# hpcaitech/Open-Sora

Measured on NVIDIA H100. Metric: denoise-steps/sec STDiT3-XL/2 64x32x32 bf16, higher is better.
Workload: dtype bf16

## Files before the change

open-sora_b200/csrc/common.cuh:

```cuda
#pragma once

#include <cuda.h>
#include <cuda_bf16.h>
#include <cuda_runtime.h>
#include <stdint.h>
#include <stdio.h>

#include "../../include/osb200.h"

namespace osb {

void set_error(const char* fmt, ...);
void count_launch(int n = 1);
bool initialised();
int sm_count();

#define OSB_CHECK_CUDA(expr)                                                            \
  do {                                                                                  \
    cudaError_t _e = (expr);                                                            \
    if (_e != cudaSuccess) {                                                            \
      osb::set_error("%s failed: %s (%s:%d)", #expr, cudaGetErrorString(_e), __FILE__,  \
                     __LINE__);                                                         \
      return OSB_ERR_CUDA;                                                              \
    }                                                                                   \
// ... 192 lines not shown
                   reinterpret_cast<uint64_t>(m)),
               "r"(src), "r"(c0), "r"(c1)
               : "memory");
}
__device__ __forceinline__ void tma_store_5d(const CUtensorMap* m, uint32_t src, int32_t c0, int32_t c1, int32_t c2,
                                             int32_t c3, int32_t c4) {
  asm volatile("cp.async.bulk.tensor.5d.global.shared::cta.bulk_group [%0, {%2, %3, %4, %5, %6}], [%1];" ::"l"(
                   reinterpret_cast<uint64_t>(m)),
               "r"(src), "r"(c0), "r"(c1), "r"(c2), "r"(c3), "r"(c4)
               : "memory");
}
__device__ __forceinline__ void bulk_commit_group() { asm volatile("cp.async.bulk.commit_group;" ::: "memory"); }
__device__ __forceinline__ void bulk_wait_group_read_all() { asm volatile("cp.async.bulk.wait_group.read 0;" ::: "memory"); }
__device__ __forceinline__ void named_barrier_sync(uint32_t id, uint32_t count) {
  asm volatile("bar.sync %0, %1;" ::"r"(id), "r"(count) : "memory");
}
__device__ __forceinline__ void wgmma_fence() { asm volatile("wgmma.fence.sync.aligned;" ::: "memory"); }
__device__ __forceinline__ void wgmma_commit() { asm volatile("wgmma.commit_group.sync.aligned;" ::: "memory"); }
template <int N>
__device__ __forceinline__ void wgmma_wait() { asm volatile("wgmma.wait_group.sync.aligned %0;" ::"n"(N) : "memory"); }
template <int R>
__device__ __forceinline__ void wgmma_fence_regs(float (&d)[R]) {
#pragma unroll
  for (int i = 0; i < R; ++i) asm volatile("" : "+f"(d[i])::"memory");
}

__device__ __forceinline__ uint64_t make_sw128_kmajor_desc(uint32_t smem_addr) {
  uint64_t d = 0;
  d |= static_cast<uint64_t>((smem_addr & 0x3FFFF) >> 4);
  d |= static_cast<uint64_t>(1) << 16;
// ... 90 lines not shown
```

open-sora_b200/csrc/gemm_sm90.cu:

```cuda
#include <stdlib.h>

#include <type_traits>

#include "common.cuh"
#include "tiles.cuh"
#include "wgmma.cuh"

namespace osb {

constexpr int kBlockM = 128;
constexpr int kBlockK = 64;
constexpr int kNumThreads = 384;
constexpr int kStageBudget = 200 * 1024;
constexpr int kSmemLimit = 227 * 1024;

enum { kPlain = 0, kConv = 1, kHeadTiles = 2, kLora = 3, kText = 4, kFp8 = 5, kFp8Blk = 6 };

struct Fp8BlockParams {
  int64_t a_ld, a_kstride;
  uint8_t* d8;
  float* d_scale;
  int64_t ldd8, ld_dscale;
};

// ... 40 lines not shown
  static constexpr int B_BYTES = BLOCK_N * kBlockK * 2;
  static constexpr int STAGE_BYTES = A_BYTES + B_BYTES;
  static constexpr int EPI_BYTES = kStaged ? kBlockM * BLOCK_N * 2 : 0;
  static constexpr int RING_BUDGET = kStaged ? kSmemLimit - 1024 - 256 - EPI_BYTES : kStageBudget;
  static constexpr int STAGES_RAW = RING_BUDGET / STAGE_BYTES;
  static constexpr int STAGES = STAGES_RAW > 6 ? 6 : STAGES_RAW;
  static constexpr int NUM_BARS = 2 * STAGES + (kStaged ? 2 : 0);
  static constexpr int SMEM_BYTES = STAGES * STAGE_BYTES + EPI_BYTES + 1024 + 8 * NUM_BARS;
  static_assert(STAGES >= 2, "pipeline needs at least two stages");
  static_assert(SMEM_BYTES <= kSmemLimit, "shared memory");
  static_assert(B_BYTES % 1024 == 0, "W tile must keep 1024-byte swizzle-atom alignment");
  static_assert(BLOCK_N % 16 == 0 && BLOCK_N <= 256, "wgmma N");
  static_assert(!kStaged || BLOCK_N % 64 == 0, "the staged epilogue moves 64-column boxes");
};

template <int BLOCK_N, int kMode>
__global__ void __launch_bounds__(kNumThreads, 1)
gemm_bf16_kernel(const __grid_constant__ CUtensorMap tmap_a, const __grid_constant__ CUtensorMap tmap_w,
                 const GemmEpilogueParams p, const ConvGeom cg, const HeadTileParams ht,
                 const __grid_constant__ CUtensorMap tmap_u, const __grid_constant__ CUtensorMap tmap_lb,
                 const int32_t lora_k_blocks,
                 const float* a_scale, const float* w_scale,
                 const Fp8BlockParams fb,
                 const __grid_constant__ CUtensorMap tmap_r,
                 const __grid_constant__ CUtensorMap tmap_d) {
  constexpr bool kStaged = staged_epilogue(kMode);
  using Cfg = GemmCfg<BLOCK_N, kStaged>;
  constexpr int kStages = Cfg::STAGES;
  constexpr int kBK = (kMode == kFp8 || kMode == kFp8Blk) ? 2 * kBlockK : kBlockK;
  constexpr uint32_t kEpiBoxBytes = kBlockM * 128;

// ... 37 lines not shown
  if (threadIdx.x == 0) {
    tma_prefetch_desc(&tmap_a);
    tma_prefetch_desc(&tmap_w);
    if constexpr (kMode == kLora) {
      tma_prefetch_desc(&tmap_u);
      tma_prefetch_desc(&tmap_lb);
    }
    if constexpr (kStaged) {
      if (p.R != nullptr) tma_prefetch_desc(&tmap_r);
      tma_prefetch_desc(&tmap_d);
      mbar_init(res_bar, 1);
      mbar_init(epi_free, 1);
    }
    for (int s = 0; s < kStages; ++s) {
      mbar_init(full_bar(s), 1);
      mbar_init(empty_bar(s), 2);
    }
    fence_barrier_init();
  }
  __syncthreads();
  pdl_wait();

  if (wg == 0) {
    asm volatile("setmaxnreg.dec.sync.aligned.u32 40;\n" ::: "memory");
    if (tid_wg == 0) {
      int stage = 0;
      uint32_t phase = 0;
      uint32_t it = 0;
      for (int64_t t = blockIdx.x; t < num_tiles; t += gridDim.x, ++it) {
        const Tile tl = tile_at(t);
        const int32_t a_row = (int32_t)(tl.m_blk * kBlockM);
        const int32_t w_row = (int32_t)(tl.n_blk * BLOCK_N);
        auto load_k_block = [&](int64_t kb) {
          mbar_wait_notrace(empty_bar(stage), phase ^ 1);
          mbar_expect_tx(full_bar(stage), Cfg::STAGE_BYTES);
          if (kMode == kLora && kb >= num_k_blocks) {
            const int32_t lk0 = (int32_t)(kb - num_k_blocks) * kBlockK;
            tma_load_2d(&tmap_u, full_bar(stage), smem_a(stage), lk0, a_row);
            tma_load_2d(&tmap_lb, full_bar(stage), smem_b(stage), lk0, w_row);
// ... 2 lines not shown
            if constexpr (kMode == kConv) {
              const int tap = (int)(kb / cg.cin_chunks);
              const int32_t ac = (int32_t)(kb - (int64_t)tap * cg.cin_chunks) * kBlockK;
              const int32_t aw = tl.w0 * cg.sw + tap % cg.kw_n;
              const int32_t ah = tl.h0 * cg.sh + (tap / cg.kw_n) % cg.kh_n;
              const int32_t at = tl.t0 * cg.st + tap / (cg.kw_n * cg.kh_n);
              tma_load_5d(&tmap_a, full_bar(stage), smem_a(stage), ac, aw, ah, at, tl.n_i);
            } else {
              tma_load_2d(&tmap_a, full_bar(stage), smem_a(stage), k0, a_row);
            }
            tma_load_2d(&tmap_w, full_bar(stage), smem_b(stage), k0, w_row);
          }
          if (++stage == kStages) { stage = 0; phase ^= 1; }
        };
        int64_t kb = 0;
        if constexpr (kStaged) {
          if (p.R != nullptr) {
            for (; kb < min((int64_t)kStages, total_k_blocks); ++kb) load_k_block(kb);
            if (it > 0) mbar_wait_notrace(epi_free, (it - 1) & 1u);
            const int live = (int)min((int64_t)(BLOCK_N / 64), (p.N - w_row + 63) / 64);
            mbar_expect_tx(res_bar, (uint32_t)live * kEpiBoxBytes);
            for (int c = 0; c < live; ++c) {
              if constexpr (kMode == kConv)
                tma_load_5d(&tmap_r, res_bar, epi_base + c * kEpiBoxBytes, w_row + 64 * c, tl.w0, tl.h0, tl.t0, tl.n_i);
              else
                tma_load_2d(&tmap_r, res_bar, epi_base + c * kEpiBoxBytes, w_row + 64 * c, a_row);
            }
          }
        }
        for (; kb < total_k_blocks; ++kb) load_k_block(kb);
      }
      pdl_launch_dependents();
    }
    return;
  }

  asm volatile("setmaxnreg.inc.sync.aligned.u32 232;\n" ::: "memory");
  const int cw = wg - 1;
  int stage = 0;
  uint32_t phase = 0;
  uint32_t it = 0;
  auto release_epi_buffer = [&](int64_t kb) {
    if constexpr (kStaged) {
      if (kb == 0 && it > 0 && threadIdx.x == 128) {
        bulk_wait_group_read_all();
        mbar_arrive(epi_free);
      }
    }
  };
  for (int64_t t = blockIdx.x; t < num_tiles; t += gridDim.x, ++it) {
    const Tile tl = tile_at(t);
    const int64_t m_blk = tl.m_blk, n_blk = tl.n_blk;
    const int warp_in = tid_wg >> 5, lane = tid_wg & 31;
    const int r_frag = cw * 64 + warp_in * 16 + (lane >> 2);
    const int c_frag = 2 * (lane & 3);
    const float* gate_row[2] = {nullptr, nullptr};
    float sa[2] = {0.f, 0.f};
    if constexpr (kStaged && kMode != kConv) {
      const uint32_t group_rows32 = (uint32_t)(p.group_rows > 0xffffffffll ? 0xffffffffu : p.group_rows);
#pragma unroll
      for (int h = 0; h < 2; ++h) {
        const int64_t row = min(m_blk * kBlockM + r_frag + 8 * h, p.M - 1);
        if (p.epilogue == OSB_EPI_BIAS_GATE_RES && p.gate != nullptr) {
          int64_t gi = (uint32_t)row / group_rows32;
          if (p.mod_index) gi = p.mod_index[gi];
          gate_row[h] = p.gate + gi * p.gate_stride;
        }
        if constexpr (kMode == kFp8) sa[h] = __ldg(a_scale + row);
      }
    }
    float acc[BLOCK_N / 2];
#pragma unroll
    for (int i = 0; i < BLOCK_N / 2; ++i) acc[i] = 0.f;
    if constexpr (kMode == kFp8 || kMode == kFp8Blk) {
      float part[BLOCK_N / 2];
#pragma unroll
      for (int i = 0; i < BLOCK_N / 2; ++i) part[i] = 0.f;
      const float* sa_row0 = a_scale;
      const float* sa_row1 = a_scale;
      if constexpr (kMode == kFp8Blk) {
        const int64_t r0 = m_blk * kBlockM + cw * 64 + (tid_wg >> 5) * 16 + ((tid_wg & 31) >> 2);
        sa_row0 = a_scale + min(r0, p.M - 1) * fb.a_ld;
        sa_row1 = a_scale + min(r0 + 8, p.M - 1) * fb.a_ld;
      }
      for (int64_t kb = 0; kb < total_k_blocks; ++kb) {
        float s0 = 1.f, s1 = 1.f;
        if constexpr (kMode == kFp8Blk) {
          s0 = __ldg(sa_row0 + kb * fb.a_kstride);
          s1 = __ldg(sa_row1 + kb * fb.a_kstride);
// ... 2 lines not shown
        const uint64_t da = make_sw128_kmajor_desc(smem_a(stage) + (uint32_t)(cw * 64 * 128));
        const uint64_t db = make_sw128_kmajor_desc(smem_b(stage));
        wgmma_fence_regs(part);
        wgmma_fence();
#pragma unroll
        for (int k = 0; k < 4; ++k)
          WgmmaFp8<BLOCK_N>::mma(part, da + (uint64_t)(2 * k), db + (uint64_t)(2 * k), k > 0 ? 1u : 0u);
        wgmma_commit();
        release_epi_buffer(kb);
        wgmma_wait<0>();
        wgmma_fence_regs(part);
        if (tid_wg == 0) mbar_arrive(empty_bar(stage));
        if constexpr (kMode == kFp8Blk) {
#pragma unroll
          for (int j = 0; j < BLOCK_N / 8; ++j) {
            acc[4 * j] = fmaf(part[4 * j], s0, acc[4 * j]);
            acc[4 * j + 1] = fmaf(part[4 * j + 1], s0, acc[4 * j + 1]);
            acc[4 * j + 2] = fmaf(part[4 * j + 2], s1, acc[4 * j + 2]);
            acc[4 * j + 3] = fmaf(part[4 * j + 3], s1, acc[4 * j + 3]);
          }
        } else {
#pragma unroll
          for (int i = 0; i < BLOCK_N / 2; ++i) acc[i] += part[i];
        }
        if (++stage == kStages) { stage = 0; phase ^= 1; }
      }
    } else {
      int prev = 0;
      for (int64_t kb = 0; kb < total_k_blocks; ++kb) {
        mbar_wait_notrace(full_bar(stage), phase);
        const uint64_t da = make_sw128_kmajor_desc(smem_a(stage) + (uint32_t)(cw * 64 * 128));
        const uint64_t db = make_sw128_kmajor_desc(smem_b(stage));
        wgmma_fence_regs(acc);
        wgmma_fence();
#pragma unroll
        for (int k = 0; k < kBlockK / 16; ++k)
          Wgmma<BLOCK_N>::mma(acc, da + (uint64_t)(2 * k), db + (uint64_t)(2 * k), (kb > 0 || k > 0) ? 1u : 0u);
        wgmma_commit();
        release_epi_buffer(kb);
        wgmma_wait<1>();
        wgmma_fence_regs(acc);
        if (kb > 0 && tid_wg == 0) mbar_arrive(empty_bar(prev));
        prev = stage;
        if (++stage == kStages) { stage = 0; phase ^= 1; }
      }
      wgmma_wait<0>();
      wgmma_fence_regs(acc);
      if (tid_wg == 0) mbar_arrive(empty_bar(prev));
    }

    if constexpr (kMode == kLora) {
      if (w_scale != nullptr) {
#pragma unroll
        for (int j = 0; j < BLOCK_N / 8; ++j) {
          const int64_t n = min(n_blk * BLOCK_N + 8 * j + c_frag, p.N - 2);
          const float2 cs = __ldg(reinterpret_cast<const float2*>(w_scale + n));
          acc[4 * j] *= cs.x;
          acc[4 * j + 1] *= cs.y;
          acc[4 * j + 2] *= cs.x;
          acc[4 * j + 3] *= cs.y;
        }
      }
    }

    if constexpr (kMode == kFp8Blk && BLOCK_N == 128) {
      if (p.epilogue == OSB_EPI_BIAS_GELU_TANH_FP8) {
        const int64_t n0 = n_blk * BLOCK_N + c_frag;
#pragma unroll
        for (int h = 0; h < 2; ++h) {
          const int64_t row = m_blk * kBlockM + r_frag + 8 * h;
          float amax = 0.f;
#pragma unroll
          for (int j = 0; j < BLOCK_N / 8; ++j) {
            const int64_t n = n0 + 8 * j;
            const float2 sw = __ldg(reinterpret_cast<const float2*>(w_scale + n));
            float v0 = acc[4 * j + 2 * h] * sw.x, v1 = acc[4 * j + 2 * h + 1] * sw.y;
            if (p.bias) {
              const float2 b = unpack_bf16x2(__ldg(reinterpret_cast<const uint32_t*>(p.bias + n)));
              v0 += b.x;
              v1 += b.y;
            }
            v0 = gelu_tanh(v0);
            v1 = gelu_tanh(v1);
            acc[4 * j + 2 * h] = v0;
            acc[4 * j + 2 * h + 1] = v1;
            amax = fmaxf(amax, fmaxf(fabsf(v0), fabsf(v1)));
          }
          amax = fmaxf(amax, __shfl_xor_sync(0xffffffffu, amax, 1));
          amax = fmaxf(amax, __shfl_xor_sync(0xffffffffu, amax, 2));
          const float s = amax > 0.f ? amax / 448.0f : 1.0f;
          if (row < p.M) {
            uint8_t* drow = fb.d8 + row * fb.ldd8;
#pragma unroll
            for (int j = 0; j < BLOCK_N / 8; ++j)
              *reinterpret_cast<uint16_t*>(drow + n0 + 8 * j) =
                  (uint16_t)e4m3x2(acc[4 * j + 2 * h] / s, acc[4 * j + 2 * h + 1] / s);
            if (c_frag == 0) fb.d_scale[row * fb.ld_dscale + n_blk] = s;
          }
        }
        continue;
      }
    }

    if constexpr (kMode == kHeadTiles) {
      constexpr int D = BLOCK_N / 2;
      using HT = HeadTileCfg<D>;
      constexpr int JH = D / 8;
      const int C = ht.heads * D;
      const uint32_t chunk_bytes = (uint32_t)ht.map.TR * 128u;
#pragma unroll
      for (int h = 0; h < 2; ++h) {
        const int64_t row = m_blk * kBlockM + r_frag + 8 * h;
        const bool row_ok = row < p.M;
        uint32_t pos = 0, tile_i = 0;
        int r = 0;
        if (row_ok) tile_of_row(ht.map, (uint32_t)row, tile_i, pos, r);
#pragma unroll
        for (int hh = 0; hh < 2; ++hh) {
          const int64_t col0 = n_blk * BLOCK_N + hh * D;
          if (col0 >= p.N) continue;
          const int kidx = (int)((uint32_t)col0 / (uint32_t)C);
          const int head = (int)((uint32_t)col0 - (uint32_t)kidx * (uint32_t)C) / D;
          const int kind = kidx % ht.nkinds;
          float x[JH][2];
#pragma unroll
          for (int j = 0; j < JH; ++j) {
            x[j][0] = acc[4 * (hh * JH + j) + 2 * h];
            x[j][1] = acc[4 * (hh * JH + j) + 2 * h + 1];
            if (p.bias) {
              const float2 b = unpack_bf16x2(__ldg(reinterpret_cast<const uint32_t*>(p.bias + col0 + 8 * j + c_frag)));
              x[j][0] += b.x;
              x[j][1] += b.y;
            }
          }
          if ((ht.norm_mask >> kind) & 1u) {
            float ss = 0.f;
#pragma unroll
            for (int j = 0; j < JH; ++j) ss += x[j][0] * x[j][0] + x[j][1] * x[j][1];
            ss += __shfl_xor_sync(0xffffffffu, ss, 1);
            ss += __shfl_xor_sync(0xffffffffu, ss, 2);
            const float rs = rsqrtf(ss * (1.0f / D) + ht.eps);
            const __nv_bfloat16* w = kind == 0 ? ht.norm_w[0] : (kind == 1 ? ht.norm_w[1] : (kind == 2 ? ht.norm_w[2] : ht.norm_w[3]));
#pragma unroll
            for (int j = 0; j < JH; ++j) {
              const float2 f = unpack_bf16x2(__ldg(reinterpret_cast<const uint32_t*>(w + 8 * j + c_frag)));
              x[j][0] *= rs * f.x;
              x[j][1] *= rs * f.y;
            }
          }
          if ((ht.rope_mask >> kind) & 1u) {
#pragma unroll
            for (int j = 0; j < JH; ++j) {
              const int64_t i = (int64_t)pos * (D / 2) + (8 * j + c_frag) / 2;
              const float cc = __ldg(ht.cos + i), sn = __ldg(ht.sin + i);
              const float a = x[j][0], b = x[j][1];
              x[j][0] = a * cc - b * sn;
              x[j][1] = b * cc + a * sn;
            }
          }
          uint8_t* dst = ht.base + (int64_t)kidx * ht.kind_stride + (int64_t)head * ht.head_stride + (int64_t)tile_i * ht.tile_bytes;
          const bool odd = (lane & 1) != 0, high = (lane & 2) != 0;
#pragma unroll
          for (int j0 = 0; j0 < HT::MAIN * 8; j0 += 4) {
            uint32_t u0 = pack_bf16x2(x[j0][0], x[j0][1]), u1 = pack_bf16x2(x[j0 + 1][0], x[j0 + 1][1]);
            uint32_t u2 = pack_bf16x2(x[j0 + 2][0], x[j0 + 2][1]), u3 = pack_bf16x2(x[j0 + 3][0], x[j0 + 3][1]);
            uint32_t s0 = __shfl_xor_sync(0xffffffffu, odd ? u0 : u1, 1);
            uint32_t s1 = __shfl_xor_sync(0xffffffffu, odd ? u2 : u3, 1);
            if (odd) { u0 = s0; u2 = s1; } else { u1 = s0; u3 = s1; }
            s0 = __shfl_xor_sync(0xffffffffu, high ? u0 : u2, 2);
            s1 = __shfl_xor_sync(0xffffffffu, high ? u1 : u3, 2);
            if (high) { u0 = s0; u1 = s1; } else { u2 = s0; u3 = s1; }
            if (row_ok)
              *reinterpret_cast<uint4*>(dst + tile_unit_off<HT::MAIN>(r, j0 + (lane & 3), chunk_bytes)) = make_uint4(u0, u1, u2, u3);
          }
          if (!row_ok) continue;
#pragma unroll
          for (int j = HT::MAIN * 8; j < JH; ++j)
            *reinterpret_cast<uint32_t*>(dst + tile_unit_off<HT::MAIN>(r, j, chunk_bytes) + c_frag * 2) = pack_bf16x2(x[j][0], x[j][1]);
          if constexpr (HT::UP > HT::U)
            *reinterpret_cast<uint32_t*>(dst + tile_unit_off<HT::MAIN>(r, HT::U, chunk_bytes) + c_frag * 2) = 0u;
        }
      }
    } else if constexpr (kMode == kText) {
#pragma unroll
      for (int h = 0; h < 2; ++h) {
        const int64_t row = m_blk * kBlockM + r_frag + 8 * h;
        if (row >= p.M) continue;
        __nv_bfloat16* drow = p.D + row * p.ldd;
#pragma unroll
        for (int j = 0; j < BLOCK_N / 8; ++j) {
          const int64_t n = n_blk * BLOCK_N + 8 * j + c_frag;
          if (n >= p.N) continue;
          float v0 = acc[4 * j + 2 * h], v1 = acc[4 * j + 2 * h + 1];
          if (p.bias) {
            const float2 b = unpack_bf16x2(__ldg(reinterpret_cast<const uint32_t*>(p.bias + n)));
            v0 += b.x;
            v1 += b.y;
          }
          if (p.epilogue == OSB_EPI_GATED_GELU) {
            drow[n >> 1] = __float2bfloat16_rn(gelu_tanh(v0) * v1);
          } else {
            v0 = v0 / (1.0f + __expf(-1.702f * v0));
            v1 = v1 / (1.0f + __expf(-1.702f * v1));
            *reinterpret_cast<uint32_t*>(drow + n) = pack_bf16x2(v0, v1);
          }
        }
      }
    } else {
      static_assert(kStaged, "every other mode has its own epilogue");
      uint8_t* const epi = smem_raw + (epi_base - smem_u32(smem_raw));
      const bool gate_res = p.epilogue == OSB_EPI_BIAS_GATE_RES;
      if (!gate_res) gate_row[0] = gate_row[1] = nullptr;
      const bool has_res = gate_res && p.R != nullptr;
      if (p.R != nullptr)
        mbar_wait_notrace(res_bar, it & 1u);
      else if (it > 0)
        mbar_wait_notrace(epi_free, (it - 1) & 1u);
      auto body = [&](auto gelu) {
#pragma unroll
        for (int j = 0; j < BLOCK_N / 8; ++j) {
          const int64_t n = min(n_blk * BLOCK_N + 8 * j + c_frag, p.N - 2);
          float2 sw = make_float2(1.f, 1.f), b = make_float2(-0.f, -0.f);
          if constexpr (kMode == kFp8 || kMode == kFp8Blk) sw = __ldg(reinterpret_cast<const float2*>(w_scale + n));
          if (p.bias) b = unpack_bf16x2(__ldg(reinterpret_cast<const uint32_t*>(p.bias + n)));
#pragma unroll
          for (int h = 0; h < 2; ++h) {
            const int li = r_frag + 8 * h;
            uint32_t* const cell = reinterpret_cast<uint32_t*>(epi + (j >> 3) * kEpiBoxBytes + li * 128 +
                                                               (((j & 7) ^ (li & 7)) << 4) + c_frag * 2);
            float v0 = acc[4 * j + 2 * h], v1 = acc[4 * j + 2 * h + 1];
            if constexpr (kMode == kFp8) {
              v0 = __fmul_rn(v0, __fmul_rn(sa[h], sw.x));
              v1 = __fmul_rn(v1, __fmul_rn(sa[h], sw.y));
            } else if constexpr (kMode == kFp8Blk) {
              v0 = __fmul_rn(v0, sw.x);
              v1 = __fmul_rn(v1, sw.y);
            }
            v0 = __fadd_rn(v0, b.x);
            v1 = __fadd_rn(v1, b.y);
            if constexpr (decltype(gelu)::value) {
              v0 = gelu_tanh(v0);
              v1 = gelu_tanh(v1);
            } else {
              const float2 g = gate_row[h] ? __ldg(reinterpret_cast<const float2*>(gate_row[h] + n)) : make_float2(1.f, 1.f);
              const float2 rv = has_res ? unpack_bf16x2(*cell) : make_float2(-0.f, -0.f);
              v0 = __fadd_rn(__fmul_rn(v0, g.x), rv.x);
              v1 = __fadd_rn(__fmul_rn(v1, g.y), rv.y);
            }
            *cell = pack_bf16x2(v0, v1);
          }
        }
      };
      if (p.epilogue == OSB_EPI_BIAS_GELU_TANH)
        body(std::true_type{});
      else
        body(std::false_type{});
      fence_proxy_async_smem();
      named_barrier_sync(1, 256);
      if (threadIdx.x == 128) {
        const int32_t n0 = (int32_t)(n_blk * BLOCK_N);
        const int live = (int)min((int64_t)(BLOCK_N / 64), (p.N - n0 + 63) / 64);
        for (int c = 0; c < live; ++c) {
          if constexpr (kMode == kConv)
            tma_store_5d(&tmap_d, epi_base + c * kEpiBoxBytes, n0 + 64 * c, tl.w0, tl.h0, tl.t0, tl.n_i);
          else
            tma_store_2d(&tmap_d, epi_base + c * kEpiBoxBytes, n0 + 64 * c, (int32_t)(m_blk * kBlockM));
        }
        bulk_commit_group();
      }
    }
  }
  if constexpr (kStaged) {
    if (threadIdx.x == 128) bulk_wait_group_read_all();
  }
}

template <int BLOCK_N, int kMode>
static int launch_kernel(const CUtensorMap& ta, const CUtensorMap& tw, const GemmEpilogueParams& p, const ConvGeom& cg,
                         const HeadTileParams& ht, int64_t tiles, cudaStream_t stream, const CUtensorMap* tu = nullptr,
                         const CUtensorMap* tlb = nullptr, int32_t lora_k_blocks = 0, const float* a_scale = nullptr,
                         const float* w_scale = nullptr, const Fp8BlockParams& fb = Fp8BlockParams{},
                         const CUtensorMap* tr = nullptr, const CUtensorMap* td = nullptr) {
  if (tiles >= (1ll << 31)) { set_error("osb gemm: too many output tiles (%lld)", (long long)tiles); return OSB_ERR_UNSUPPORTED; }
  const int64_t grid = tiles < sm_count() ? tiles : sm_count();
  cudaLaunchAttribute attr[2];
  cudaLaunchConfig_t cfg = launch_config(dim3((unsigned)grid), dim3(kNumThreads),
                                         GemmCfg<BLOCK_N, staged_epilogue(kMode)>::SMEM_BYTES, stream, attr);
  OSB_CHECK_CUDA(cudaLaunchKernelEx(&cfg, gemm_bf16_kernel<BLOCK_N, kMode>, ta, tw, p, cg, ht, tu ? *tu : ta,
                                    tlb ? *tlb : tw, lora_k_blocks, a_scale, w_scale, fb, tr ? *tr : ta, td ? *td : ta));
  count_launch();
  return OSB_OK;
}

static int make_epilogue_maps(const GemmEpilogueParams& p, CUtensorMap* tr, CUtensorMap* td) {
  if (int rc = make_tmap_2d_bf16(td, p.D, p.M, p.N, p.ldd, kBlockM, 64)) return rc;
  if (p.R != nullptr) return make_tmap_2d_bf16(tr, p.R, p.M, p.N, p.ldr, kBlockM, 64);
  *tr = *td;
  return OSB_OK;
}

template <int D>
static int launch_gemm_ht(const osb_gemm_args& a, const HeadTileParams& ht, cudaStream_t stream) {
  constexpr int BLOCK_N = 2 * D;
  CUtensorMap ta, tw;
// ... 36 lines not shown
  if (lora == nullptr && a.epilogue >= OSB_EPI_GATED_GELU) return launch_kernel<BLOCK_N, kText>(ta, tw, p, cg, ht, tiles, stream);
  CUtensorMap tr, td;
  if ((rc = make_epilogue_maps(p, &tr, &td))) return rc;
  if (lora == nullptr)
    return launch_kernel<BLOCK_N, kPlain>(ta, tw, p, cg, ht, tiles, stream, nullptr, nullptr, 0, nullptr, nullptr,
                                          Fp8BlockParams{}, &tr, &td);
  CUtensorMap tu, tlb;
  if ((rc = make_tmap_2d_bf16(&tu, lora->U, a.M, lora->r, lora->ldu, kBlockM, kBlockK))) return rc;
  if ((rc = make_tmap_2d_bf16(&tlb, lora->B, a.N, lora->r, lora->ldb, BLOCK_N, kBlockK))) return rc;
  return launch_kernel<BLOCK_N, kLora>(ta, tw, p, cg, ht, tiles, stream, &tu, &tlb, (lora->r + kBlockK - 1) / kBlockK,
                                       nullptr, lora->col_scale, Fp8BlockParams{}, &tr, &td);
}

template <int BLOCK_N, int kMode>
static int init_one() {
  OSB_CHECK_CUDA(cudaFuncSetAttribute(gemm_bf16_kernel<BLOCK_N, kMode>, cudaFuncAttributeMaxDynamicSharedMemorySize,
                                      GemmCfg<BLOCK_N, staged_epilogue(kMode)>::SMEM_BYTES));
  return OSB_OK;
}

int gemm_init() {
  int rc = 0;
  if ((rc = init_one<128, kHeadTiles>())) return rc;
  if ((rc = init_one<144, kHeadTiles>())) return rc;
  if ((rc = init_one<256, kHeadTiles>())) return rc;
  if ((rc = init_one<64, kPlain>())) return rc;
  if ((rc = init_one<128, kPlain>())) return rc;
  if ((rc = init_one<192, kPlain>())) return rc;
  if ((rc = init_one<256, kPlain>())) return rc;
  if ((rc = init_one<64, kConv>())) return rc;
  if ((rc = init_one<128, kConv>())) return rc;
  if ((rc = init_one<192, kConv>())) return rc;
// ... 1 lines not shown
  if ((rc = init_one<64, kLora>())) return rc;
  if ((rc = init_one<128, kLora>())) return rc;
  if ((rc = init_one<192, kLora>())) return rc;
  if ((rc = init_one<256, kLora>())) return rc;
  if ((rc = init_one<64, kText>())) return rc;
  if ((rc = init_one<128, kText>())) return rc;
  if ((rc = init_one<192, kText>())) return rc;
  if ((rc = init_one<256, kText>())) return rc;
  if ((rc = init_one<64, kFp8>())) return rc;
  if ((rc = init_one<128, kFp8>())) return rc;
  if ((rc = init_one<64, kFp8Blk>())) return rc;
  if ((rc = init_one<128, kFp8Blk>())) return rc;
  return OSB_OK;
}

static int pick_block_n(int64_t M, int64_t N) {
  if (N <= 64) return 64;
  const int cands[3] = {256, 192, 128};
  int best = 256;
  int64_t best_cost = INT64_MAX;
  for (int i = 0; i < 3; ++i) {
    const int bn = cands[i];
    const int64_t tiles = ((M + kBlockM - 1) / kBlockM) * ((N + bn - 1) / bn);
    const int64_t waves = (tiles + sm_count() - 1) / sm_count();
    const int64_t cost = waves * (bn + 16);
    if (cost < best_cost) { best_cost = cost; best = bn; }
  }
  return best;
}

template <int BLOCK_N, int kMode = kFp8>
static int launch_gemm_fp8(const osb_gemm_fp8_args& a, cudaStream_t stream, const Fp8BlockParams& fb = Fp8BlockParams{}) {
  CUtensorMap ta, tw;
  int rc = make_tmap_2d_e4m3(&ta, a.A, a.M, a.K, a.lda, kBlockM, 2 * kBlockK);
  if (rc) return rc;
  rc = make_tmap_2d_e4m3(&tw, a.W, a.N, a.K, a.ldw, BLOCK_N, 2 * kBlockK);
  if (rc) return rc;
  GemmEpilogueParams p = {};
  p.bias = static_cast<const __nv_bfloat16*>(a.bias);
  p.D = static_cast<__nv_bfloat16*>(a.D);
// ... 82 lines not shown
  }
  OSB_REQUIRE(a.bias == nullptr || (reinterpret_cast<uintptr_t>(a.bias) & 15) == 0,
              "%s: bias must be 16-byte aligned", fn);
  OSB_REQUIRE(a.cta_group >= 0 && a.cta_group <= 2, "%s: cta_group must be 0, 1 or 2", fn);
  if (lora != nullptr) {
    const osb_lora_args& l = *lora;
    OSB_REQUIRE(l.U && l.B, "%s: null U or B", fn);
    OSB_REQUIRE(l.r > 0 && l.r % 8 == 0, "%s: rank r must be a positive multiple of 8 (zero-pad A and B), got %d", fn, l.r);
    OSB_REQUIRE(l.ldu >= l.r && l.ldb >= l.r && l.ldu % 8 == 0 && l.ldb % 8 == 0 &&
                ((reinterpret_cast<uintptr_t>(l.U) | reinterpret_cast<uintptr_t>(l.B)) & 15) == 0,
                "%s: U and B must be 16-byte aligned with ldu, ldb >= r and multiples of 8 (r %d ldu %lld ldb %lld)", fn,
                l.r, (long long)l.ldu, (long long)l.ldb);
    OSB_REQUIRE((reinterpret_cast<uintptr_t>(l.col_scale) & 7) == 0, "%s: col_scale must be 8-byte aligned", fn);
  }
  const bool has_res = (a.epilogue == OSB_EPI_BIAS_GATE_RES) && a.R != nullptr;
  const int bn = a.block_n ? a.block_n : pick_block_n(a.M, a.N);
  cudaStream_t s = static_cast<cudaStream_t>(stream);
  if (bn == 64) return launch_gemm<64>(a, has_res, s, lora);
  if (bn == 128) return launch_gemm<128>(a, has_res, s, lora);
  if (bn == 192) return launch_gemm<192>(a, has_res, s, lora);
  if (bn == 256) return launch_gemm<256>(a, has_res, s, lora);
  set_error("%s: unsupported block_n %d", fn, bn);
  return OSB_ERR_UNSUPPORTED;
}

}

extern "C" int osb_gemm_bf16(const osb_gemm_args* args, void* stream) {
  return osb::gemm_dispatch("osb_gemm_bf16", args, nullptr, stream);
}

// ... 197 lines not shown
```

Before: 12.17.

## Add ping-pong consumer schedule to plain and head-tile bf16 GEMMs

For plain and head-tile GEMMs with block_n up to 192, the two consumer warpgroups each take a whole 128-row tile in alternation instead of splitting one tile. Ordering is enforced with named barriers so one warpgroup's epilogue overlaps the other's MMA mainloop. Register allocation shifts further toward the consumers, and the staged epilogue now issues its own residual load and frees the buffer per warpgroup. The block_n picker also changes to a K-weighted cost model with a separate epilogue term, which may select different tile widths. This raises per-thread register use to two accumulator sets and adds barrier and phase-tracking complexity.

```diff
diff --git a/open-sora_b200/csrc/common.cuh b/open-sora_b200/csrc/common.cuh
--- a/open-sora_b200/csrc/common.cuh
+++ b/open-sora_b200/csrc/common.cuh
@@ -230,6 +230,9 @@
 __device__ __forceinline__ void bulk_wait_group_read_all() { asm volatile("cp.async.bulk.wait_group.read 0;" ::: "memory"); }
 __device__ __forceinline__ void named_barrier_sync(uint32_t id, uint32_t count) {
   asm volatile("bar.sync %0, %1;" ::"r"(id), "r"(count) : "memory");
+}
+__device__ __forceinline__ void named_barrier_arrive(uint32_t id, uint32_t count) {
+  asm volatile("bar.arrive %0, %1;" ::"r"(id), "r"(count) : "memory");
 }
 __device__ __forceinline__ void wgmma_fence() { asm volatile("wgmma.fence.sync.aligned;" ::: "memory"); }
 __device__ __forceinline__ void wgmma_commit() { asm volatile("wgmma.commit_group.sync.aligned;" ::: "memory"); }
diff --git a/open-sora_b200/csrc/gemm_sm90.cu b/open-sora_b200/csrc/gemm_sm90.cu
--- a/open-sora_b200/csrc/gemm_sm90.cu
+++ b/open-sora_b200/csrc/gemm_sm90.cu
@@ -78,7 +78,11 @@
   static_assert(!kStaged || BLOCK_N % 64 == 0, "the staged epilogue moves 64-column boxes");
 };
 
-template <int BLOCK_N, int kMode>
+__host__ __device__ constexpr bool pingpong_schedule(int block_n, int mode) {
+  return (mode == kPlain || mode == kHeadTiles) && block_n <= 192;
+}
+
+template <int BLOCK_N, int kMode, bool kPingPong>
 __global__ void __launch_bounds__(kNumThreads, 1)
 gemm_bf16_kernel(const __grid_constant__ CUtensorMap tmap_a, const __grid_constant__ CUtensorMap tmap_w,
                  const GemmEpilogueParams p, const ConvGeom cg, const HeadTileParams ht,
@@ -146,7 +150,7 @@
     }
     for (int s = 0; s < kStages; ++s) {
       mbar_init(full_bar(s), 1);
-      mbar_init(empty_bar(s), 2);
+      mbar_init(empty_bar(s), kPingPong ? 1 : 2);
     }
     fence_barrier_init();
   }
@@ -154,7 +158,10 @@
   pdl_wait();
 
   if (wg == 0) {
-    asm volatile("setmaxnreg.dec.sync.aligned.u32 40;\n" ::: "memory");
+    if constexpr (kPingPong)
+      asm volatile("setmaxnreg.dec.sync.aligned.u32 24;\n" ::: "memory");
+    else
+      asm volatile("setmaxnreg.dec.sync.aligned.u32 40;\n" ::: "memory");
     if (tid_wg == 0) {
       int stage = 0;
       uint32_t phase = 0;
@@ -187,7 +194,7 @@
           if (++stage == kStages) { stage = 0; phase ^= 1; }
         };
         int64_t kb = 0;
-        if constexpr (kStaged) {
+        if constexpr (kStaged && !kPingPong) {
           if (p.R != nullptr) {
             for (; kb < min((int64_t)kStages, total_k_blocks); ++kb) load_k_block(kb);
             if (it > 0) mbar_wait_notrace(epi_free, (it - 1) & 1u);
@@ -208,44 +215,73 @@
     return;
   }
 
-  asm volatile("setmaxnreg.inc.sync.aligned.u32 232;\n" ::: "memory");
+  if constexpr (kPingPong)
+    asm volatile("setmaxnreg.inc.sync.aligned.u32 240;\n" ::: "memory");
+  else
+    asm volatile("setmaxnreg.inc.sync.aligned.u32 232;\n" ::: "memory");
+  constexpr int kHalves = kPingPong ? 2 : 1;
   const int cw = wg - 1;
   int stage = 0;
   uint32_t phase = 0;
-  uint32_t it = 0;
+  uint32_t it = kPingPong ? cw : 0;
   auto release_epi_buffer = [&](int64_t kb) {
-    if constexpr (kStaged) {
+    if constexpr (kStaged && !kPingPong) {
       if (kb == 0 && it > 0 && threadIdx.x == 128) {
         bulk_wait_group_read_all();
         mbar_arrive(epi_free);
       }
     }
   };
-  for (int64_t t = blockIdx.x; t < num_tiles; t += gridDim.x, ++it) {
-    const Tile tl = tile_at(t);
-    const int64_t m_blk = tl.m_blk, n_blk = tl.n_blk;
+  auto grid_ctas = [&]() -> uint32_t {
+    if constexpr (!kPingPong) return gridDim.x;
+    uint32_t n;
+    asm volatile("mov.u32 %0, %%nctaid.x;" : "=r"(n));
+    return n;
+  };
+  for (int64_t t = blockIdx.x + (int64_t)it * grid_ctas(); t < num_tiles; t += kHalves * grid_ctas(), it += kHalves) {
+    Tile tl = {};
+    int64_t m_blk = 0, n_blk = 0;
+    auto locate = [&]() {
+      tl = tile_at(t);
+      m_blk = tl.m_blk;
+      n_blk = tl.n_blk;
+    };
+    if constexpr (!kPingPong) locate();
     const int warp_in = tid_wg >> 5, lane = tid_wg & 31;
-    const int r_frag = cw * 64 + warp_in * 16 + (lane >> 2);
+    auto r_frag = [&](int mh) { return (kPingPong ? mh : cw) * 64 + warp_in * 16 + (lane >> 2); };
     const int c_frag = 2 * (lane & 3);
-    const float* gate_row[2] = {nullptr, nullptr};
+    if constexpr (kPingPong) {
+      const uint64_t pos = (uint64_t)it * (uint64_t)total_k_blocks;
+      stage = (int)(pos % kStages);
+      phase = (uint32_t)(pos / kStages) & 1u;
+    }
+    const float* gate_row[kHalves][2] = {};
     float sa[2] = {0.f, 0.f};
-    if constexpr (kStaged && kMode != kConv) {
+    auto row_operands = [&]() {
       const uint32_t group_rows32 = (uint32_t)(p.group_rows > 0xffffffffll ? 0xffffffffu : p.group_rows);
 #pragma unroll
-      for (int h = 0; h < 2; ++h) {
-        const int64_t row = min(m_blk * kBlockM + r_frag + 8 * h, p.M - 1);
-        if (p.epilogue == OSB_EPI_BIAS_GATE_RES && p.gate != nullptr) {
-          int64_t gi = (uint32_t)row / group_rows32;
-          if (p.mod_index) gi = p.mod_index[gi];
-          gate_row[h] = p.gate + gi * p.gate_stride;
-        }
-        if constexpr (kMode == kFp8) sa[h] = __ldg(a_scale + row);
-      }
-    }
-    float acc[BLOCK_N / 2];
-#pragma unroll
-    for (int i = 0; i < BLOCK_N / 2; ++i) acc[i] = 0.f;
+      for (int mh = 0; mh < kHalves; ++mh) {
+#pragma unroll
+        for (int h = 0; h < 2; ++h) {
+          const int64_t row = min(m_blk * kBlockM + r_frag(mh) + 8 * h, p.M - 1);
+          if (p.epilogue == OSB_EPI_BIAS_GATE_RES && p.gate != nullptr) {
+            int64_t gi = (uint32_t)row / group_rows32;
+            if (p.mod_index) gi = p.mod_index[gi];
+            gate_row[mh][h] = p.gate + gi * p.gate_stride;
+          }
+          if constexpr (kMode == kFp8) sa[h] = __ldg(a_scale + row);
+        }
+      }
+    };
+    if constexpr (kStaged && kMode != kConv && !kPingPong) row_operands();
+    float acc[kHalves][BLOCK_N / 2];
+#pragma unroll
+    for (int mh = 0; mh < kHalves; ++mh) {
+#pragma unroll
+      for (int i = 0; i < BLOCK_N / 2; ++i) acc[mh][i] = 0.f;
+    }
     if constexpr (kMode == kFp8 || kMode == kFp8Blk) {
+      static_assert(!kPingPong, "the FP8 modes run the cooperative schedule");
       float part[BLOCK_N / 2];
 #pragma unroll
       for (int i = 0; i < BLOCK_N / 2; ++i) part[i] = 0.f;
@@ -278,40 +314,54 @@
         if constexpr (kMode == kFp8Blk) {
 #pragma unroll
           for (int j = 0; j < BLOCK_N / 8; ++j) {
-            acc[4 * j] = fmaf(part[4 * j], s0, acc[4 * j]);
-            acc[4 * j + 1] = fmaf(part[4 * j + 1], s0, acc[4 * j + 1]);
-            acc[4 * j + 2] = fmaf(part[4 * j + 2], s1, acc[4 * j + 2]);
-            acc[4 * j + 3] = fmaf(part[4 * j + 3], s1, acc[4 * j + 3]);
+            acc[0][4 * j] = fmaf(part[4 * j], s0, acc[0][4 * j]);
+            acc[0][4 * j + 1] = fmaf(part[4 * j + 1], s0, acc[0][4 * j + 1]);
+            acc[0][4 * j + 2] = fmaf(part[4 * j + 2], s1, acc[0][4 * j + 2]);
+            acc[0][4 * j + 3] = fmaf(part[4 * j + 3], s1, acc[0][4 * j + 3]);
           }
         } else {
 #pragma unroll
-          for (int i = 0; i < BLOCK_N / 2; ++i) acc[i] += part[i];
+          for (int i = 0; i < BLOCK_N / 2; ++i) acc[0][i] += part[i];
         }
         if (++stage == kStages) { stage = 0; phase ^= 1; }
       }
     } else {
+      if constexpr (kPingPong) {
+        if (it > 0) named_barrier_sync(3 + cw, 256);
+      }
       int prev = 0;
       for (int64_t kb = 0; kb < total_k_blocks; ++kb) {
         mbar_wait_notrace(full_bar(stage), phase);
-        const uint64_t da = make_sw128_kmajor_desc(smem_a(stage) + (uint32_t)(cw * 64 * 128));
+        const uint64_t da = make_sw128_kmajor_desc(smem_a(stage) + (uint32_t)(kPingPong ? 0 : cw * 64 * 128));
         const uint64_t db = make_sw128_kmajor_desc(smem_b(stage));
-        wgmma_fence_regs(acc);
+#pragma unroll
+        for (int mh = 0; mh < kHalves; ++mh) wgmma_fence_regs(acc[mh]);
         wgmma_fence();
 #pragma unroll
-        for (int k = 0; k < kBlockK / 16; ++k)
-          Wgmma<BLOCK_N>::mma(acc, da + (uint64_t)(2 * k), db + (uint64_t)(2 * k), (kb > 0 || k > 0) ? 1u : 0u);
+        for (int k = 0; k < kBlockK / 16; ++k) {
+#pragma unroll
+          for (int mh = 0; mh < kHalves; ++mh)
+            Wgmma<BLOCK_N>::mma(acc[mh], da + (uint64_t)(512 * mh + 2 * k), db + (uint64_t)(2 * k),
+                                (kb > 0 || k > 0) ? 1u : 0u);
+        }
         wgmma_commit();
         release_epi_buffer(kb);
         wgmma_wait<1>();
-        wgmma_fence_regs(acc);
+#pragma unroll
+        for (int mh = 0; mh < kHalves; ++mh) wgmma_fence_regs(acc[mh]);
         if (kb > 0 && tid_wg == 0) mbar_arrive(empty_bar(prev));
         prev = stage;
         if (++stage == kStages) { stage = 0; phase ^= 1; }
       }
+      if constexpr (kPingPong) {
+        if (t + grid_ctas() < num_tiles) named_barrier_arrive(3 + (cw ^ 1), 256);
+      }
       wgmma_wait<0>();
-      wgmma_fence_regs(acc);
+#pragma unroll
+      for (int mh = 0; mh < kHalves; ++mh) wgmma_fence_regs(acc[mh]);
       if (tid_wg == 0) mbar_arrive(empty_bar(prev));
     }
+    if constexpr (kPingPong) locate();
 
     if constexpr (kMode == kLora) {
       if (w_scale != nullptr) {
@@ -319,10 +369,10 @@
         for (int j = 0; j < BLOCK_N / 8; ++j) {
           const int64_t n = min(n_blk * BLOCK_N + 8 * j + c_frag, p.N - 2);
           const float2 cs = __ldg(reinterpret_cast<const float2*>(w_scale + n));
-          acc[4 * j] *= cs.x;
-          acc[4 * j + 1] *= cs.y;
-          acc[4 * j + 2] *= cs.x;
-          acc[4 * j + 3] *= cs.y;
+          acc[0][4 * j] *= cs.x;
+          acc[0][4 * j + 1] *= cs.y;
+          acc[0][4 * j + 2] *= cs.x;
+          acc[0][4 * j + 3] *= cs.y;
         }
       }
     }
@@ -332,13 +382,13 @@
         const int64_t n0 = n_blk * BLOCK_N + c_frag;
 #pragma unroll
         for (int h = 0; h < 2; ++h) {
-          const int64_t row = m_blk * kBlockM + r_frag + 8 * h;
+          const int64_t row = m_blk * kBlockM + r_frag(0) + 8 * h;
           float amax = 0.f;
 #pragma unroll
           for (int j = 0; j < BLOCK_N / 8; ++j) {
             const int64_t n = n0 + 8 * j;
             const float2 sw = __ldg(reinterpret_cast<const float2*>(w_scale + n));
-            float v0 = acc[4 * j + 2 * h] * sw.x, v1 = acc[4 * j + 2 * h + 1] * sw.y;
+            float v0 = acc[0][4 * j + 2 * h] * sw.x, v1 = acc[0][4 * j + 2 * h + 1] * sw.y;
             if (p.bias) {
               const float2 b = unpack_bf16x2(__ldg(reinterpret_cast<const uint32_t*>(p.bias + n)));
               v0 += b.x;
@@ -346,8 +396,8 @@
             }
             v0 = gelu_tanh(v0);
             v1 = gelu_tanh(v1);
-            acc[4 * j + 2 * h] = v0;
-            acc[4 * j + 2 * h + 1] = v1;
+            acc[0][4 * j + 2 * h] = v0;
+            acc[0][4 * j + 2 * h + 1] = v1;
             amax = fmaxf(amax, fmaxf(fabsf(v0), fabsf(v1)));
           }
           amax = fmaxf(amax, __shfl_xor_sync(0xffffffffu, amax, 1));
@@ -358,7 +408,7 @@
 #pragma unroll
             for (int j = 0; j < BLOCK_N / 8; ++j)
               *reinterpret_cast<uint16_t*>(drow + n0 + 8 * j) =
-                  (uint16_t)e4m3x2(acc[4 * j + 2 * h] / s, acc[4 * j + 2 * h + 1] / s);
+                  (uint16_t)e4m3x2(acc[0][4 * j + 2 * h] / s, acc[0][4 * j + 2 * h + 1] / s);
             if (c_frag == 0) fb.d_scale[row * fb.ld_dscale + n_blk] = s;
           }
         }
@@ -373,89 +423,93 @@
       const int C = ht.heads * D;
       const uint32_t chunk_bytes = (uint32_t)ht.map.TR * 128u;
 #pragma unroll
+      for (int mh = 0; mh < kHalves; ++mh) {
+#pragma unroll
+        for (int h = 0; h < 2; ++h) {
+          const int64_t row = m_blk * kBlockM + r_frag(mh) + 8 * h;
+          const bool row_ok = row < p.M;
+          uint32_t pos = 0, tile_i = 0;
+          int r = 0;
+          if (row_ok) tile_of_row(ht.map, (uint32_t)row, tile_i, pos, r);
+#pragma unroll
+          for (int hh = 0; hh < 2; ++hh) {
+            const int64_t col0 = n_blk * BLOCK_N + hh * D;
+            if (col0 >= p.N) continue;
+            const int kidx = (int)((uint32_t)col0 / (uint32_t)C);
+            const int head = (int)((uint32_t)col0 - (uint32_t)kidx * (uint32_t)C) / D;
+            const int kind = kidx % ht.nkinds;
+            float x[JH][2];
+#pragma unroll
+            for (int j = 0; j < JH; ++j) {
+              x[j][0] = acc[mh][4 * (hh * JH + j) + 2 * h];
+              x[j][1] = acc[mh][4 * (hh * JH + j) + 2 * h + 1];
+              if (p.bias) {
+                const float2 b = unpack_bf16x2(__ldg(reinterpret_cast<const uint32_t*>(p.bias + col0 + 8 * j + c_frag)));
+                x[j][0] += b.x;
+                x[j][1] += b.y;
+              }
+            }
+            if ((ht.norm_mask >> kind) & 1u) {
+              float ss = 0.f;
+#pragma unroll
+              for (int j = 0; j < JH; ++j) ss += x[j][0] * x[j][0] + x[j][1] * x[j][1];
+              ss += __shfl_xor_sync(0xffffffffu, ss, 1);
+              ss += __shfl_xor_sync(0xffffffffu, ss, 2);
+              const float rs = rsqrtf(ss * (1.0f / D) + ht.eps);
+              const __nv_bfloat16* w = kind == 0 ? ht.norm_w[0] : (kind == 1 ? ht.norm_w[1] : (kind == 2 ? ht.norm_w[2] : ht.norm_w[3]));
+#pragma unroll
+              for (int j = 0; j < JH; ++j) {
+                const float2 f = unpack_bf16x2(__ldg(reinterpret_cast<const uint32_t*>(w + 8 * j + c_frag)));
+                x[j][0] *= rs * f.x;
+                x[j][1] *= rs * f.y;
+              }
+            }
+            if ((ht.rope_mask >> kind) & 1u) {
+#pragma unroll
+              for (int j = 0; j < JH; ++j) {
+                const int64_t i = (int64_t)pos * (D / 2) + (8 * j + c_frag) / 2;
+                const float cc = __ldg(ht.cos + i), sn = __ldg(ht.sin + i);
+                const float a = x[j][0], b = x[j][1];
+                x[j][0] = a * cc - b * sn;
+                x[j][1] = b * cc + a * sn;
+              }
+            }
+            uint8_t* dst = ht.base + (int64_t)kidx * ht.kind_stride + (int64_t)head * ht.head_stride + (int64_t)tile_i * ht.tile_bytes;
+            const bool odd = (lane & 1) != 0, high = (lane & 2) != 0;
+#pragma unroll
+            for (int j0 = 0; j0 < HT::MAIN * 8; j0 += 4) {
+              uint32_t u0 = pack_bf16x2(x[j0][0], x[j0][1]), u1 = pack_bf16x2(x[j0 + 1][0], x[j0 + 1][1]);
+              uint32_t u2 = pack_bf16x2(x[j0 + 2][0], x[j0 + 2][1]), u3 = pack_bf16x2(x[j0 + 3][0], x[j0 + 3][1]);
+              uint32_t s0 = __shfl_xor_sync(0xffffffffu, odd ? u0 : u1, 1);
+              uint32_t s1 = __shfl_xor_sync(0xffffffffu, odd ? u2 : u3, 1);
+              if (odd) { u0 = s0; u2 = s1; } else { u1 = s0; u3 = s1; }
+              s0 = __shfl_xor_sync(0xffffffffu, high ? u0 : u2, 2);
+              s1 = __shfl_xor_sync(0xffffffffu, high ? u1 : u3, 2);
+              if (high) { u0 = s0; u1 = s1; } else { u2 = s0; u3 = s1; }
+              if (row_ok)
+                *reinterpret_cast<uint4*>(dst + tile_unit_off<HT::MAIN>(r, j0 + (lane & 3), chunk_bytes)) = make_uint4(u0, u1, u2, u3);
+            }
+            if (!row_ok) continue;
+#pragma unroll
+            for (int j = HT::MAIN * 8; j < JH; ++j)
+              *reinterpret_cast<uint32_t*>(dst + tile_unit_off<HT::MAIN>(r, j, chunk_bytes) + c_frag * 2) = pack_bf16x2(x[j][0], x[j][1]);
+            if constexpr (HT::UP > HT::U)
+              *reinterpret_cast<uint32_t*>(dst + tile_unit_off<HT::MAIN>(r, HT::U, chunk_bytes) + c_frag * 2) = 0u;
+          }
+        }
+      }
+    } else if constexpr (kMode == kText) {
+      static_assert(!kPingPong, "the text mode runs the cooperative schedule");
+#pragma unroll
       for (int h = 0; h < 2; ++h) {
-        const int64_t row = m_blk * kBlockM + r_frag + 8 * h;
-        const bool row_ok = row < p.M;
-        uint32_t pos = 0, tile_i = 0;
-        int r = 0;
-        if (row_ok) tile_of_row(ht.map, (uint32_t)row, tile_i, pos, r);
-#pragma unroll
-        for (int hh = 0; hh < 2; ++hh) {
-          const int64_t col0 = n_blk * BLOCK_N + hh * D;
-          if (col0 >= p.N) continue;
-          const int kidx = (int)((uint32_t)col0 / (uint32_t)C);
-          const int head = (int)((uint32_t)col0 - (uint32_t)kidx * (uint32_t)C) / D;
-          const int kind = kidx % ht.nkinds;
-          float x[JH][2];
-#pragma unroll
-          for (int j = 0; j < JH; ++j) {
-            x[j][0] = acc[4 * (hh * JH + j) + 2 * h];
-            x[j][1] = acc[4 * (hh * JH + j) + 2 * h + 1];
-            if (p.bias) {
-              const float2 b = unpack_bf16x2(__ldg(reinterpret_cast<const uint32_t*>(p.bias + col0 + 8 * j + c_frag)));
-              x[j][0] += b.x;
-              x[j][1] += b.y;
-            }
-          }
-          if ((ht.norm_mask >> kind) & 1u) {
-            float ss = 0.f;
-#pragma unroll
-            for (int j = 0; j < JH; ++j) ss += x[j][0] * x[j][0] + x[j][1] * x[j][1];
-            ss += __shfl_xor_sync(0xffffffffu, ss, 1);
-            ss += __shfl_xor_sync(0xffffffffu, ss, 2);
-            const float rs = rsqrtf(ss * (1.0f / D) + ht.eps);
-            const __nv_bfloat16* w = kind == 0 ? ht.norm_w[0] : (kind == 1 ? ht.norm_w[1] : (kind == 2 ? ht.norm_w[2] : ht.norm_w[3]));
-#pragma unroll
-            for (int j = 0; j < JH; ++j) {
-              const float2 f = unpack_bf16x2(__ldg(reinterpret_cast<const uint32_t*>(w + 8 * j + c_frag)));
-              x[j][0] *= rs * f.x;
-              x[j][1] *= rs * f.y;
-            }
-          }
-          if ((ht.rope_mask >> kind) & 1u) {
-#pragma unroll
-            for (int j = 0; j < JH; ++j) {
-              const int64_t i = (int64_t)pos * (D / 2) + (8 * j + c_frag) / 2;
-              const float cc = __ldg(ht.cos + i), sn = __ldg(ht.sin + i);
-              const float a = x[j][0], b = x[j][1];
-              x[j][0] = a * cc - b * sn;
-              x[j][1] = b * cc + a * sn;
-            }
-          }
-          uint8_t* dst = ht.base + (int64_t)kidx * ht.kind_stride + (int64_t)head * ht.head_stride + (int64_t)tile_i * ht.tile_bytes;
-          const bool odd = (lane & 1) != 0, high = (lane & 2) != 0;
-#pragma unroll
-          for (int j0 = 0; j0 < HT::MAIN * 8; j0 += 4) {
-            uint32_t u0 = pack_bf16x2(x[j0][0], x[j0][1]), u1 = pack_bf16x2(x[j0 + 1][0], x[j0 + 1][1]);
-            uint32_t u2 = pack_bf16x2(x[j0 + 2][0], x[j0 + 2][1]), u3 = pack_bf16x2(x[j0 + 3][0], x[j0 + 3][1]);
-            uint32_t s0 = __shfl_xor_sync(0xffffffffu, odd ? u0 : u1, 1);
-            uint32_t s1 = __shfl_xor_sync(0xffffffffu, odd ? u2 : u3, 1);
-            if (odd) { u0 = s0; u2 = s1; } else { u1 = s0; u3 = s1; }
-            s0 = __shfl_xor_sync(0xffffffffu, high ? u0 : u2, 2);
-            s1 = __shfl_xor_sync(0xffffffffu, high ? u1 : u3, 2);
-            if (high) { u0 = s0; u1 = s1; } else { u2 = s0; u3 = s1; }
-            if (row_ok)
-              *reinterpret_cast<uint4*>(dst + tile_unit_off<HT::MAIN>(r, j0 + (lane & 3), chunk_bytes)) = make_uint4(u0, u1, u2, u3);
-          }
-          if (!row_ok) continue;
-#pragma unroll
-          for (int j = HT::MAIN * 8; j < JH; ++j)
-            *reinterpret_cast<uint32_t*>(dst + tile_unit_off<HT::MAIN>(r, j, chunk_bytes) + c_frag * 2) = pack_bf16x2(x[j][0], x[j][1]);
-          if constexpr (HT::UP > HT::U)
-            *reinterpret_cast<uint32_t*>(dst + tile_unit_off<HT::MAIN>(r, HT::U, chunk_bytes) + c_frag * 2) = 0u;
-        }
-      }
-    } else if constexpr (kMode == kText) {
-#pragma unroll
-      for (int h = 0; h < 2; ++h) {
-        const int64_t row = m_blk * kBlockM + r_frag + 8 * h;
+        const int64_t row = m_blk * kBlockM + r_frag(0) + 8 * h;
         if (row >= p.M) continue;
         __nv_bfloat16* drow = p.D + row * p.ldd;
 #pragma unroll
         for (int j = 0; j < BLOCK_N / 8; ++j) {
           const int64_t n = n_blk * BLOCK_N + 8 * j + c_frag;
           if (n >= p.N) continue;
-          float v0 = acc[4 * j + 2 * h], v1 = acc[4 * j + 2 * h + 1];
+          float v0 = acc[0][4 * j + 2 * h], v1 = acc[0][4 * j + 2 * h + 1];
           if (p.bias) {
             const float2 b = unpack_bf16x2(__ldg(reinterpret_cast<const uint32_t*>(p.bias + n)));
             v0 += b.x;
@@ -473,45 +527,79 @@
     } else {
       static_assert(kStaged, "every other mode has its own epilogue");
       uint8_t* const epi = smem_raw + (epi_base - smem_u32(smem_raw));
+      if constexpr (kPingPong) row_operands();
       const bool gate_res = p.epilogue == OSB_EPI_BIAS_GATE_RES;
-      if (!gate_res) gate_row[0] = gate_row[1] = nullptr;
+      if (!gate_res) {
+#pragma unroll
+        for (int mh = 0; mh < kHalves; ++mh) gate_row[mh][0] = gate_row[mh][1] = nullptr;
+      }
       const bool has_res = gate_res && p.R != nullptr;
-      if (p.R != nullptr)
-        mbar_wait_notrace(res_bar, it & 1u);
-      else if (it > 0)
-        mbar_wait_notrace(epi_free, (it - 1) & 1u);
+      int32_t n0 = 0;
+      int live = 0;
+      auto boxes = [&]() {
+        n0 = (int32_t)(n_blk * BLOCK_N);
+        live = (int)min((int64_t)(BLOCK_N / 64), (p.N - n0 + 63) / 64);
+      };
+      if constexpr (kPingPong) {
+        if (it > 0) mbar_wait_notrace(epi_free, (it - 1) & 1u);
+        if (p.R != nullptr) {
+          if (tid_wg == 0) {
+            const int32_t c0 = (int32_t)(n_blk * BLOCK_N);
+            uint32_t bytes = 0;
+#pragma unroll
+            for (int c = 0; c < BLOCK_N / 64; ++c)
+              if (c0 + 64 * c < p.N) bytes += kEpiBoxBytes;
+            mbar_expect_tx(res_bar, bytes);
+#pragma unroll
+            for (int c = 0; c < BLOCK_N / 64; ++c)
+              if (c0 + 64 * c < p.N)
+                tma_load_2d(&tmap_r, res_bar, epi_base + c * kEpiBoxBytes, c0 + 64 * c, (int32_t)(m_blk * kBlockM));
+          }
+          mbar_wait_notrace(res_bar, it & 1u);
+        }
+      } else {
+        if (p.R != nullptr)
+          mbar_wait_notrace(res_bar, it & 1u);
+        else if (it > 0)
+          mbar_wait_notrace(epi_free, (it - 1) & 1u);
+      }
       auto body = [&](auto gelu) {
 #pragma unroll
         for (int j = 0; j < BLOCK_N / 8; ++j) {
-          const int64_t n = min(n_blk * BLOCK_N + 8 * j + c_frag, p.N - 2);
+          const int64_t n = kPingPong ? (int64_t)min((int32_t)(n_blk * BLOCK_N) + 8 * j + c_frag, (int32_t)p.N - 2)
+                                      : min(n_blk * BLOCK_N + 8 * j + c_frag, p.N - 2);
           float2 sw = make_float2(1.f, 1.f), b = make_float2(-0.f, -0.f);
           if constexpr (kMode == kFp8 || kMode == kFp8Blk) sw = __ldg(reinterpret_cast<const float2*>(w_scale + n));
           if (p.bias) b = unpack_bf16x2(__ldg(reinterpret_cast<const uint32_t*>(p.bias + n)));
 #pragma unroll
-          for (int h = 0; h < 2; ++h) {
-            const int li = r_frag + 8 * h;
-            uint32_t* const cell = reinterpret_cast<uint32_t*>(epi + (j >> 3) * kEpiBoxBytes + li * 128 +
-                                                               (((j & 7) ^ (li & 7)) << 4) + c_frag * 2);
-            float v0 = acc[4 * j + 2 * h], v1 = acc[4 * j + 2 * h + 1];
-            if constexpr (kMode == kFp8) {
-              v0 = __fmul_rn(v0, __fmul_rn(sa[h], sw.x));
-              v1 = __fmul_rn(v1, __fmul_rn(sa[h], sw.y));
-            } else if constexpr (kMode == kFp8Blk) {
-              v0 = __fmul_rn(v0, sw.x);
-              v1 = __fmul_rn(v1, sw.y);
+          for (int mh = 0; mh < kHalves; ++mh) {
+#pragma unroll
+            for (int h = 0; h < 2; ++h) {
+              const int li = r_frag(mh) + 8 * h;
+              uint32_t* const cell = reinterpret_cast<uint32_t*>(epi + (j >> 3) * kEpiBoxBytes + li * 128 +
+                                                                 (((j & 7) ^ (li & 7)) << 4) + c_frag * 2);
+              float v0 = acc[mh][4 * j + 2 * h], v1 = acc[mh][4 * j + 2 * h + 1];
+              if constexpr (kMode == kFp8) {
+                v0 = __fmul_rn(v0, __fmul_rn(sa[h], sw.x));
+                v1 = __fmul_rn(v1, __fmul_rn(sa[h], sw.y));
+              } else if constexpr (kMode == kFp8Blk) {
+                v0 = __fmul_rn(v0, sw.x);
+                v1 = __fmul_rn(v1, sw.y);
+              }
+              v0 = __fadd_rn(v0, b.x);
+              v1 = __fadd_rn(v1, b.y);
+              if constexpr (decltype(gelu)::value) {
+                v0 = gelu_tanh(v0);
+                v1 = gelu_tanh(v1);
+              } else {
+                const float* const gr = gate_row[mh][h];
+                const float2 g = gr ? __ldg(reinterpret_cast<const float2*>(gr + n)) : make_float2(1.f, 1.f);
+                const float2 rv = has_res ? unpack_bf16x2(*cell) : make_float2(-0.f, -0.f);
+                v0 = __fadd_rn(__fmul_rn(v0, g.x), rv.x);
+                v1 = __fadd_rn(__fmul_rn(v1, g.y), rv.y);
+              }
+              *cell = pack_bf16x2(v0, v1);
             }
-            v0 = __fadd_rn(v0, b.x);
-            v1 = __fadd_rn(v1, b.y);
-            if constexpr (decltype(gelu)::value) {
-              v0 = gelu_tanh(v0);
-              v1 = gelu_tanh(v1);
-            } else {
-              const float2 g = gate_row[h] ? __ldg(reinterpret_cast<const float2*>(gate_row[h] + n)) : make_float2(1.f, 1.f);
-              const float2 rv = has_res ? unpack_bf16x2(*cell) : make_float2(-0.f, -0.f);
-              v0 = __fadd_rn(__fmul_rn(v0, g.x), rv.x);
-              v1 = __fadd_rn(__fmul_rn(v1, g.y), rv.y);
-            }
-            *cell = pack_bf16x2(v0, v1);
           }
         }
       };
@@ -520,21 +608,30 @@
       else
         body(std::false_type{});
       fence_proxy_async_smem();
-      named_barrier_sync(1, 256);
-      if (threadIdx.x == 128) {
-        const int32_t n0 = (int32_t)(n_blk * BLOCK_N);
-        const int live = (int)min((int64_t)(BLOCK_N / 64), (p.N - n0 + 63) / 64);
+      named_barrier_sync(kPingPong ? 1 + cw : 1, kPingPong ? 128 : 256);
+      if (kPingPong ? tid_wg == 0 : threadIdx.x == 128) {
+        if constexpr (kPingPong) {
+          n0 = (int32_t)(n_blk * BLOCK_N);
+          live = BLOCK_N / 64;
+        } else {
+          boxes();
+        }
         for (int c = 0; c < live; ++c) {
+          if (kPingPong && n0 + 64 * c >= p.N) break;
           if constexpr (kMode == kConv)
             tma_store_5d(&tmap_d, epi_base + c * kEpiBoxBytes, n0 + 64 * c, tl.w0, tl.h0, tl.t0, tl.n_i);
           else
             tma_store_2d(&tmap_d, epi_base + c * kEpiBoxBytes, n0 + 64 * c, (int32_t)(m_blk * kBlockM));
         }
         bulk_commit_group();
-      }
-    }
-  }
-  if constexpr (kStaged) {
+        if constexpr (kPingPong) {
+          bulk_wait_group_read_all();
+          mbar_arrive(epi_free);
+        }
+      }
+    }
+  }
+  if constexpr (kStaged && !kPingPong) {
     if (threadIdx.x == 128) bulk_wait_group_read_all();
   }
 }
@@ -550,8 +647,9 @@
   cudaLaunchAttribute attr[2];
   cudaLaunchConfig_t cfg = launch_config(dim3((unsigned)grid), dim3(kNumThreads),
                                          GemmCfg<BLOCK_N, staged_epilogue(kMode)>::SMEM_BYTES, stream, attr);
-  OSB_CHECK_CUDA(cudaLaunchKernelEx(&cfg, gemm_bf16_kernel<BLOCK_N, kMode>, ta, tw, p, cg, ht, tu ? *tu : ta,
-                                    tlb ? *tlb : tw, lora_k_blocks, a_scale, w_scale, fb, tr ? *tr : ta, td ? *td : ta));
+  OSB_CHECK_CUDA(cudaLaunchKernelEx(&cfg, gemm_bf16_kernel<BLOCK_N, kMode, pingpong_schedule(BLOCK_N, kMode)>, ta, tw,
+                                    p, cg, ht, tu ? *tu : ta, tlb ? *tlb : tw, lora_k_blocks, a_scale, w_scale, fb,
+                                    tr ? *tr : ta, td ? *td : ta));
   count_launch();
   return OSB_OK;
 }
@@ -618,8 +716,8 @@
 
 template <int BLOCK_N, int kMode>
 static int init_one() {
-  OSB_CHECK_CUDA(cudaFuncSetAttribute(gemm_bf16_kernel<BLOCK_N, kMode>, cudaFuncAttributeMaxDynamicSharedMemorySize,
-                                      GemmCfg<BLOCK_N, staged_epilogue(kMode)>::SMEM_BYTES));
+  OSB_CHECK_CUDA(cudaFuncSetAttribute(gemm_bf16_kernel<BLOCK_N, kMode, pingpong_schedule(BLOCK_N, kMode)>,
+                                      cudaFuncAttributeMaxDynamicSharedMemorySize, GemmCfg<BLOCK_N, staged_epilogue(kMode)>::SMEM_BYTES));
   return OSB_OK;
 }
 
@@ -651,7 +749,7 @@
   return OSB_OK;
 }
 
-static int pick_block_n(int64_t M, int64_t N) {
+static int pick_block_n(int64_t M, int64_t N, int64_t K) {
   if (N <= 64) return 64;
   const int cands[3] = {256, 192, 128};
   int best = 256;
@@ -660,7 +758,8 @@
     const int bn = cands[i];
     const int64_t tiles = ((M + kBlockM - 1) / kBlockM) * ((N + bn - 1) / bn);
     const int64_t waves = (tiles + sm_count() - 1) / sm_count();
-    const int64_t cost = waves * (bn + 16);
+    constexpr int64_t kEpi = 16 * 1152;
+    const int64_t cost = bn == 192 ? waves * 198 * K + kEpi : bn == 256 ? waves * (bn * K + kEpi) : waves * (bn + 16) * K;
     if (cost < best_cost) { best_cost = cost; best = bn; }
   }
   return best;
@@ -773,7 +872,7 @@
     OSB_REQUIRE((reinterpret_cast<uintptr_t>(l.col_scale) & 7) == 0, "%s: col_scale must be 8-byte aligned", fn);
   }
   const bool has_res = (a.epilogue == OSB_EPI_BIAS_GATE_RES) && a.R != nullptr;
-  const int bn = a.block_n ? a.block_n : pick_block_n(a.M, a.N);
+  const int bn = a.block_n ? a.block_n : pick_block_n(a.M, a.N, a.K);
   cudaStream_t s = static_cast<cudaStream_t>(stream);
   if (bn == 64) return launch_gemm<64>(a, has_res, s, lora);
   if (bn == 128) return launch_gemm<128>(a, has_res, s, lora);
```

Result: faster. 12.40, median of 6 (+1.9%).
